# GAIR-Lab/IISAN

Measured on AMD Instinct MI355X. Metric: items/s (fwd+bwd) ViT-B+BERT-B IISAN uncached, Scientific, bs=128, higher is better.
Workload: dtype fp16; 1 GPU; Code_Uncached IISAN ViT-base+BERT-base, Amazon-Scientific-shaped synthetic batch, bs=128/GPU (1408 item slots, all encoded), 1xMI355X per rank; global_batch=128, parallelism=dp1, encoder_blocks=all tokens in every block

## Files before the change

### iisan_amd/csrc/attn16.hip

```cpp
#include "common.h"
#ifndef ATTN_KBATCH
#define ATTN_KBATCH 4
#endif

#ifdef ATTN_DEBUG_BITS
static int g_attn_dbg = 0;
IISAN_DEV_KNOB(attn_debug, g_attn_dbg);
#else
static constexpr int g_attn_dbg = 0;
#endif

namespace {

constexpr float MASK_RAW = -0x1p126f;

template <typename T> struct Mfma16k16;
template <> struct Mfma16k16<F16> {
    static __device__ __forceinline__ f4 run(h4 a, h4 b, f4 c) { return __builtin_amdgcn_mfma_f32_16x16x16f16(a, b, c, 0, 0, 0); }
};
template <> struct Mfma16k16<BF16> {
    typedef short s4 __attribute__((ext_vector_type(4)));
    static __device__ __forceinline__ f4 run(b4 a, b4 b, f4 c) {
        return __builtin_amdgcn_mfma_f32_16x16x16bf16_1k(__builtin_bit_cast(s4, a), __builtin_bit_cast(s4, b), c, 0, 0, 0);
    }
};

template <typename T, int NT16, bool PF, bool MASKALL>
__global__ __launch_bounds__(256, PF ? 2 : 3) void attention16_kernel(const typename T::elem* __restrict__ qkv,
                                                             const float* __restrict__ key_bias,
                                                             typename T::elem* __restrict__ ctx, int S, int heads, int hpw,
                                                             int dbg_arg) {
    typedef typename T::elem E;
    typedef typename T::v8 V8;
    typedef typename T::v4 V4;
#ifndef ATTN_DEBUG_BITS
    (void)dbg_arg;
    constexpr int dbg = 0;
#else
    const int dbg = dbg_arg;
#endif
    constexpr int SP = NT16 * 16;
    constexpr int VT_LD = 32 * ((NT16 + 1) / 2) + 16;
    constexpr int MAXQB = (NT16 + 3) / 4;
    constexpr int KP = (SP + 31) / 32;
    constexpr int VP = (SP / 4 + 31) / 32;
    __shared__ __attribute__((aligned(16))) char smem[SP * 128 + 64 * VT_LD * 2 + SP * 4];
    char* sK = smem;
    E* sVt = (E*)(smem + SP * 128);
    float* sKB = (float*)(smem + SP * 128 + 64 * VT_LD * 2);

    const int tid = threadIdx.x, lane = tid & 63, wave = tid >> 6;
    const int groups = heads / hpw;
    const int item = blockIdx.x / groups, h0 = (blockIdx.x - item * groups) * hpw;
    const int D = heads * 64;
    const int j = lane & 15, g = lane >> 4;
    const int nqb = (S + 15) >> 4;
    const int c = tid & 7, r0 = tid >> 3;

    V8 kreg[KP], vreg[VP][4], qnext[MAXQB][2];
    auto load_head = [&](int h) {
        if (dbg & 32) return;
        const E* qb_ = qkv + ((int64_t)item * heads + h) * 3 * S * 64;
        const E* kb_ = qb_ + (int64_t)S * 64;
        const E* vb_ = kb_ + (int64_t)S * 64;
        int t2 = tid;
        asm volatile("" : "+v"(t2));
        const int wave = t2 >> 6, j = t2 & 15, g = (t2 >> 4) & 3, c = t2 & 7, r0 = t2 >> 3;
#pragma unroll
        for (int i = 0; i < MAXQB; ++i) {
            int sq = (wave + 4 * i) * 16 + j;
            sq = sq < S ? sq : S - 1;
#pragma unroll
            for (int kk = 0; kk < 2; ++kk) qnext[i][kk] = *(const V8*)(qb_ + (unsigned)(sq * 64 + kk * 32 + g * 8));
        }
#pragma unroll
        for (int p = 0; p < KP; ++p) {
            const int r = r0 + 32 * p;
            kreg[p] = __builtin_nontemporal_load((const V8*)(kb_ + (unsigned)((r < S ? r : S - 1) * 64 + c * 8)));
        }
#pragma unroll
        for (int p = 0; p < VP; ++p)
#pragma unroll
            for (int r = 0; r < 4; ++r) {
                const int key = (r0 + 32 * p) * 4 + r;
                if (SP > 64 || r0 + 32 * p < SP / 4) vreg[p][r] = __builtin_nontemporal_load((const V8*)(vb_ + (unsigned)((key < S ? key : S - 1) * 64 + c * 8)));
            }
    };

    if (PF) load_head(h0);
    for (int r = tid; r < SP; r += 256)
        sKB[r] = r >= S ? -INFINITY : ((key_bias && key_bias[(int64_t)item * S + r] < 0.f) ? MASK_RAW : INFINITY);

    const float c2 = 0.18033688011112042f;
#pragma unroll 1
    for (int hi = 0; hi < hpw; ++hi) {
        const int h = h0 + hi;
        if (!PF) load_head(h);
        if (hi > 0) __syncthreads();
#pragma unroll
        for (int p = 0; p < KP; ++p) {
            const int r = r0 + 32 * p;
            if ((SP % 32 == 0 || r < SP) && !(dbg & 16)) *(V8*)(sK + r * 128 + ((c ^ (r & 7)) << 4)) = kreg[p];
        }
#pragma unroll
        for (int p = 0; p < VP; ++p) {
            const int kg = r0 + 32 * p;
            if (kg < SP / 4) {
#pragma unroll
                for (int e = 0; e < 8; ++e) {
                    V4 t;
#pragma unroll
                    for (int r = 0; r < 4; ++r) t[r] = vreg[p][r][e];
                    if (!(dbg & 1)) *(V4*)(sVt + (c * 8 + e) * VT_LD + 32 * (kg >> 3) + 8 * (kg & 3) + 4 * ((kg >> 2) & 1)) = t;
                }
            }
        }
        V8 qf[MAXQB][2];
#pragma unroll
        for (int i = 0; i < MAXQB; ++i)
#pragma unroll
            for (int kk = 0; kk < 2; ++kk) qf[i][kk] = qnext[i][kk];
        __syncthreads();
        if (PF && hi + 1 < hpw) load_head(h + 1);

#pragma unroll
        for (int i = 0; i < MAXQB; ++i) {
            const int qb = wave + 4 * i;
            if (qb >= nqb || (dbg & 64)) break;
            const int sq = qb * 16 + j;

            f4 sc[NT16];
            {
                constexpr int KBATCH = NT16 >= 13 ? ATTN_KBATCH : (NT16 % 4 == 0 ? 4 : NT16);
#pragma unroll
                for (int t0 = 0; t0 < NT16; t0 += KBATCH) {
                    V8 kf[KBATCH][2];
#pragma unroll
                    for (int u = 0; u < KBATCH; ++u)
#pragma unroll
                        for (int kk = 0; kk < 2; ++kk)
                            if (t0 + u < NT16) kf[u][kk] = *(const V8*)(sK + ((t0 + u) * 16 + j) * 128 + (((kk * 4 + g) ^ (j & 7)) << 4));
                    __builtin_amdgcn_sched_barrier(0);
#pragma unroll
                    for (int u = 0; u < KBATCH; ++u) {
                        if (t0 + u >= NT16) continue;
                        f4 acc = {0.f, 0.f, 0.f, 0.f};
                        acc = T::mfma(kf[u][0], qf[i][0], acc);
                        acc = T::mfma(kf[u][1], qf[i][1], acc);
                        sc[t0 + u] = acc;
                    }
                }
            }
#pragma unroll
            for (int t = 0; t < NT16; ++t) {
                if (MASKALL || t == NT16 - 1) {
                    const f4 kb = *(const f4*)(sKB + t * 16 + g * 4);
#pragma unroll
                    for (int r = 0; r < 4; ++r) sc[t][r] = __builtin_amdgcn_fmed3f(sc[t][r], kb[r], -INFINITY);
                }
            }
            float mx0 = -INFINITY, mx1 = -INFINITY;
#pragma unroll
            for (int t = 0; t < NT16; ++t) {
                if (t & 1) mx1 = fmaxf(fmaxf(mx1, sc[t][0]), fmaxf(sc[t][1], fmaxf(sc[t][2], sc[t][3])));
                else mx0 = fmaxf(fmaxf(mx0, sc[t][0]), fmaxf(sc[t][1], fmaxf(sc[t][2], sc[t][3])));
            }
            float mx = fmaxf(mx0, mx1);
            mx = fmaxf(mx, __shfl_xor(mx, 16, 64));
            mx = fmaxf(mx, __shfl_xor(mx, 32, 64));
            f4 sum4 = {0.f, 0.f, 0.f, 0.f};
            const float mxs = -(mx * c2);
#pragma unroll
            for (int t = 0; t < NT16; ++t)
#pragma unroll
                for (int r = 0; r < 4; ++r) {
                    const float a = fmaf(sc[t][r], c2, mxs);
                    const float p = __builtin_amdgcn_exp2f(a);
                    sc[t][r] = p;
                    sum4[r] += p;
                }
            float sum = (sum4[0] + sum4[1]) + (sum4[2] + sum4[3]);
            sum += __shfl_xor(sum, 16, 64);
            sum += __shfl_xor(sum, 32, 64);
            const float inv = 1.0f / sum;

            f4 o[4];
#pragma unroll
            for (int dt = 0; dt < 4; ++dt) o[dt] = (f4){0.f, 0.f, 0.f, 0.f};
            {
                auto vload = [&](int kb, V8 (&vf)[4]) {
#pragma unroll
                    for (int dt = 0; dt < 4; ++dt) vf[dt] = *(const V8*)(sVt + (dt * 16 + j) * VT_LD + kb * 32 + g * 8);
                };
                V8 vc[4];
                vload(0, vc);
                constexpr int NPV = NT16 / 2;
#pragma unroll
                for (int kb = 0; kb < NPV; ++kb) {
                    V8 vn[4];
                    if (kb + 1 < NPV) vload(kb + 1, vn);
                    V8 pf;
#pragma unroll
                    for (int e = 0; e < 4; ++e) {
                        pf[e] = T::from_f32(sc[2 * kb][e]);
                        pf[4 + e] = T::from_f32(sc[2 * kb + 1][e]);
                    }
#pragma unroll
                    for (int dt = 0; dt < 4; ++dt) o[dt] = T::mfma(vc[dt], pf, o[dt]);
                    if (kb + 1 < NPV) {
#pragma unroll
                        for (int dt = 0; dt < 4; ++dt) vc[dt] = vn[dt];
                    }
                }
                if constexpr (NT16 % 2 == 1) {
                    V4 pt;
#pragma unroll
                    for (int e = 0; e < 4; ++e) pt[e] = T::from_f32(sc[NT16 - 1][e]);
#pragma unroll
                    for (int dt = 0; dt < 4; ++dt)
                        o[dt] = Mfma16k16<T>::run(*(const V4*)(sVt + (dt * 16 + j) * VT_LD + (NT16 / 2) * 32 + g * 8), pt, o[dt]);
                }
            }
            typedef unsigned u2 __attribute__((ext_vector_type(2)));
            u2 pk[4];
#pragma unroll
            for (int dt = 0; dt < 4; ++dt) {
                V4 ov;
#pragma unroll
                for (int r = 0; r < 4; ++r) ov[r] = T::from_f32(o[dt][r] * inv);
                pk[dt] = __builtin_bit_cast(u2, ov);
            }
#pragma unroll
            for (int q2 = 0; q2 < 2; ++q2)
#pragma unroll
                for (int w = 0; w < 2; ++w) {
                    const auto sw = __builtin_amdgcn_permlane16_swap(pk[2 * q2][w], pk[2 * q2 + 1][w], false, false);
                    pk[2 * q2][w] = sw[0];
                    pk[2 * q2 + 1][w] = sw[1];
                }
            if (sq < S && !(dbg & 8)) {
                int g2 = g;
                asm volatile("" : "+v"(g2));
                E* op = ctx + (size_t)item * S * D + (unsigned)(sq * D + h * 64 + g2 * 4 + ((g2 & 1) ? 12 : 0));
                typedef unsigned u4 __attribute__((ext_vector_type(4)));
#pragma unroll
                for (int q2 = 0; q2 < 2; ++q2)
                    *(u4*)(op + q2 * 32) = (u4){pk[2 * q2][0], pk[2 * q2][1], pk[2 * q2 + 1][0], pk[2 * q2 + 1][1]};
            }
        }
    }
}

template <typename T>
__global__ __launch_bounds__(256) void attention_cls_kernel(const typename T::elem* __restrict__ qkv,
                                                            const float* __restrict__ key_bias,
                                                            typename T::elem* __restrict__ ctx, int64_t pairs, int S, int heads,
                                                            const typename T::elem* __restrict__ q_cls) {
    typedef typename T::elem E;
    typedef typename T::v8 V8;
    typedef typename T::v4 V4;
    __shared__ float sP[4][256];
    const int lane = threadIdx.x & 63, wave = threadIdx.x >> 6;
    const int64_t pair = (int64_t)blockIdx.x * 4 + wave;
    if (pair >= pairs) return;
    const int64_t item = pair / heads;
    const int h = (int)(pair - item * heads);
    const E* qb_ = qkv + pair * 3 * S * 64;
    const E* kb_ = qb_ + (int64_t)S * 64;
    const E* vb_ = kb_ + (int64_t)S * 64;
    const int kc = lane & 7, kr = lane >> 3;
    float q[8];
    {
        const V8 t = q_cls ? *(const V8*)(q_cls + (item * heads + h) * 64 + kc * 8) : *(const V8*)(qb_ + kc * 8);
#pragma unroll
        for (int e = 0; e < 8; ++e) q[e] = T::to_f32(t[e]);
    }
    float mx = -INFINITY;
    constexpr int KB = 5;
    for (int k0 = 0; k0 < S; k0 += 8 * KB) {
        V8 t[KB];
        float kbv[KB];
#pragma unroll
        for (int u = 0; u < KB; ++u) {
            const int key = k0 + 8 * u + kr;
            const int kcl = key < S ? key : S - 1;
            t[u] = *(const V8*)(kb_ + (int64_t)kcl * 64 + kc * 8);
            kbv[u] = key_bias ? key_bias[item * S + kcl] : 0.f;
        }
#pragma unroll
        for (int u = 0; u < KB; ++u) {
            const int key = k0 + 8 * u + kr;
            float a = 0.f;
#pragma unroll
            for (int e = 0; e < 8; ++e) a = fmaf(q[e], T::to_f32(t[u][e]), a);
            a += __shfl_xor(a, 1, 64);
            a += __shfl_xor(a, 2, 64);
            a += __shfl_xor(a, 4, 64);
            if (key >= S) a = -INFINITY;
            else if (kbv[u] < 0.f) a = MASK_RAW;
            if (kc == 0 && key < 256) sP[wave][key] = a;
            mx = fmaxf(mx, a);
        }
    }
#pragma unroll
    for (int o = 8; o < 64; o <<= 1) mx = fmaxf(mx, __shfl_xor(mx, o, 64));
    __builtin_amdgcn_s_waitcnt(0xc07f);
    const float c2 = 0.18033688011112042f;
    float sum = 0.f;
#pragma unroll
    for (int i = 0; i < 4; ++i) {
        const int key = lane + 64 * i;
        const float a = key < S ? sP[wave][key] : -INFINITY;
        const float p = __builtin_amdgcn_exp2f((a - mx) * c2);
        sum += p;
        sP[wave][key] = T::to_f32(T::from_f32(p));
    }
#pragma unroll
    for (int o = 1; o < 64; o <<= 1) sum += __shfl_xor(sum, o, 64);
    const float inv = 1.0f / sum;
    __builtin_amdgcn_s_waitcnt(0xc07f);
    const int kg = lane >> 4, dq = lane & 15;
    float acc[4] = {0.f, 0.f, 0.f, 0.f};
    constexpr int VB = 8;
    for (int k0 = kg; k0 < S; k0 += 4 * VB) {
        V4 v[VB];
        float pr[VB];
#pragma unroll
        for (int u = 0; u < VB; ++u) {
            const int key = k0 + 4 * u;
            const int kcl = key < S ? key : S - 1;
            v[u] = *(const V4*)(vb_ + (int64_t)kcl * 64 + dq * 4);
            pr[u] = key < S ? sP[wave][kcl] : 0.f;
        }
#pragma unroll
        for (int u = 0; u < VB; ++u)
#pragma unroll
            for (int e = 0; e < 4; ++e) acc[e] = fmaf(pr[u], T::to_f32(v[u][e]), acc[e]);
    }
#pragma unroll
    for (int e = 0; e < 4; ++e) {
        acc[e] += __shfl_xor(acc[e], 16, 64);
        acc[e] += __shfl_xor(acc[e], 32, 64);
    }
    if (kg == 0) {
        V4 o;
#pragma unroll
        for (int e = 0; e < 4; ++e) o[e] = T::from_f32(acc[e] * inv);
        *(V4*)(ctx + item * (int64_t)heads * 64 + h * 64 + dq * 4) = o;
    }
}

template <typename T>
int launch_t(const void* qkv, const float* key_bias, void* ctx, int64_t items, int S, int heads, hipStream_t s) {
    typedef typename T::elem E;
    int hpw = heads % 2 == 0 ? 2 : 1;
#ifdef ATTN_DEBUG_BITS
    {
        const int want = (g_attn_dbg >> 8) & 15;
        if (want > 0 && heads % want == 0) hpw = want;
    }
#endif
    dim3 grid((unsigned)(items * (heads / hpw))), block(256);
#define IISAN_ATTN_CASE(NT)                                                                                                       \
    if (key_bias == nullptr && S > 16 * (NT - 1))                                                                                 \
        hipLaunchKernelGGL((attention16_kernel<T, NT, true, false>), grid, block, 0, s, (const E*)qkv, key_bias, (E*)ctx, S, heads, hpw, g_attn_dbg & 127); \
    else                                                                                                                          \
        hipLaunchKernelGGL((attention16_kernel<T, NT, true, true>), grid, block, 0, s, (const E*)qkv, key_bias, (E*)ctx, S, heads, hpw, g_attn_dbg & 127)
    if (S <= 32) { IISAN_ATTN_CASE(2); }
    else if (S <= 64) { IISAN_ATTN_CASE(4); }
    else if (S <= 128) { IISAN_ATTN_CASE(8); }
    else if (S <= 208) { IISAN_ATTN_CASE(13); }
    else if (S <= 224) { IISAN_ATTN_CASE(14); }
    else {
        iisan_set_error("attention16: sequence length %d > 224 not supported", S);
        return IISAN_EBADSHAPE;
    }
#undef IISAN_ATTN_CASE
    IISAN_LAUNCH_OK();
    return IISAN_OK;
}

}

int launch_attention16(int dtype16, const void* qkv, const float* key_bias, void* ctx, int64_t items, int S, int heads,
                       hipStream_t s) {
    IISAN_CHECK_SHAPE(items > 0 && S > 0 && heads > 0, "attention16: empty problem");
    IISAN_CHECK_SHAPE(items * heads < (1ll << 31), "attention16: grid too large");
    IISAN_CHECK_SHAPE((int64_t)S * heads * 64 < (1ll << 31), "attention16: item of %d x %d elements too large", S, heads * 64);
    return dtype16 == IISAN_BF16 ? launch_t<BF16>(qkv, key_bias, ctx, items, S, heads, s)
                                 : launch_t<F16>(qkv, key_bias, ctx, items, S, heads, s);
}

int launch_attention_cls16(int dtype16, const void* qkv, const float* key_bias, void* ctx_cls, int64_t items, int S, int heads,
                           hipStream_t s, const void* q_cls) {
    IISAN_CHECK_SHAPE(items > 0 && S > 0 && S <= 256 && heads > 0, "attention_cls16: unsupported problem (S=%d)", S);
    const int64_t pairs = items * heads;
    dim3 grid((unsigned)ceil_div(pairs, 4)), block(256);
    if (dtype16 == IISAN_BF16)
        hipLaunchKernelGGL(attention_cls_kernel<BF16>, grid, block, 0, s, (const __bf16*)qkv, key_bias, (__bf16*)ctx_cls, pairs, S, heads, (const __bf16*)q_cls);
    else
        hipLaunchKernelGGL(attention_cls_kernel<F16>, grid, block, 0, s, (const _Float16*)qkv, key_bias, (_Float16*)ctx_cls, pairs, S, heads, (const _Float16*)q_cls);
    IISAN_LAUNCH_OK();
    return IISAN_OK;
}

extern "C" int iisan_attention16(int32_t dtype16, const void* qkv, const float* key_bias, void* ctx, int64_t items,
                                 int32_t S, int32_t heads, void* stream) {
    return launch_attention16(dtype16, qkv, key_bias, ctx, items, S, heads, (hipStream_t)stream);
}

extern "C" int iisan_attention_cls16(int32_t dtype16, const void* qkv, const float* key_bias, void* ctx_cls, int64_t items,
                                     int32_t S, int32_t heads, void* stream) {
    return launch_attention_cls16(dtype16, qkv, key_bias, ctx_cls, items, S, heads, (hipStream_t)stream, nullptr);
}
```

### iisan_amd/csrc/common.h

```cpp
#pragma once

#include <hip/hip_runtime.h>
#include <stdint.h>
#include <stdio.h>
#include <string.h>

#include "../../include/iisan_hip.h"

typedef _Float16 h8 __attribute__((ext_vector_type(8)));
typedef _Float16 h4 __attribute__((ext_vector_type(4)));
typedef __bf16 b8 __attribute__((ext_vector_type(8)));
typedef __bf16 b4 __attribute__((ext_vector_type(4)));
typedef float f4 __attribute__((ext_vector_type(4)));
typedef unsigned int u4 __attribute__((ext_vector_type(4)));
typedef unsigned int u2 __attribute__((ext_vector_type(2)));

#define WAVE 64

void iisan_set_error(const char* fmt, ...);

#define IISAN_CHECK_SHAPE(cond, ...)                                                                             \
    do {                                                                                                         \
        if (!(cond)) {                                                                                           \
            iisan_set_error(__VA_ARGS__);                                                                        \
            return IISAN_EBADSHAPE;                                                                              \
        }                                                                                                        \
    } while (0)

#define IISAN_HIP_OK(expr)                                                                                       \
    do {                                                                                                         \
        hipError_t _e = (expr);                                                                                  \
        if (_e != hipSuccess) {                                                                                  \
            iisan_set_error("%s failed at %s:%d: %s", #expr, __FILE__, __LINE__, hipGetErrorString(_e));         \
            return IISAN_EHIP;                                                                                   \
        }                                                                                                        \
    } while (0)

#define IISAN_LAUNCH_OK() IISAN_HIP_OK(hipGetLastError())

struct IisanDevKnob {
    const char* name;
    int64_t def;
    int64_t (*get)();
    void (*set)(int64_t);
};
int iisan_dev_register(const IisanDevKnob& k);
#define IISAN_DEV_KNOB(NAME, VAR)                                                                                \
    static const int iisan_dev_reg_##NAME = iisan_dev_register(IisanDevKnob{                                     \
        #NAME, (int64_t)(VAR), [] { return (int64_t)(VAR); }, [](int64_t v) { VAR = (decltype(VAR))v; }})
#define IISAN_DEV_COUNTER(NAME, VAR)                                                                             \
    static const int iisan_dev_cnt_##NAME = iisan_dev_register(IisanDevKnob{                                     \
        "count:" #NAME, INT64_MIN, [] { return (int64_t)(VAR); }, [](int64_t v) { VAR = (decltype(VAR))v; }})
#define IISAN_DEV_KNOB_FN(NAME, VAR, SET)                                                                        \
    static const int iisan_dev_reg_##NAME = iisan_dev_register(IisanDevKnob{                                     \
        #NAME, (int64_t)(VAR), [] { return (int64_t)(VAR); }, [](int64_t v) { SET; }})

#define IISAN_TRY(expr)                                                                                          \
    do {                                                                                                         \
        int _r = (expr);                                                                                         \
        if (_r != IISAN_OK) return _r;                                                                           \
    } while (0)

constexpr int IISAN_MAX_DEVICES = 64;
int iisan_cu_count();
struct OncePerDevice {
    bool done[IISAN_MAX_DEVICES] = {};
    bool first() {
        int dev = 0;
        if (hipGetDevice(&dev) != hipSuccess || dev < 0 || dev >= IISAN_MAX_DEVICES) return true;
        if (done[dev]) return false;
        done[dev] = true;
        return true;
    }
};

static inline size_t align_up(size_t x, size_t a) { return (x + a - 1) / a * a; }
static inline int64_t ceil_div(int64_t a, int64_t b) { return (a + b - 1) / b; }

struct WsCarver {
    char* base;
    size_t cap, off;
    bool overflow;
    WsCarver(void* p, size_t n) : base((char*)p), cap(n), off(0), overflow(false) {}
    template <typename T>
    T* take(size_t count) {
        size_t bytes = align_up(count * sizeof(T), 256);
        if (base && off + bytes > cap) overflow = true;
        T* r = base ? (T*)(base + off) : nullptr;
        off += bytes;
        return r;
    }
};

struct F16 {
    typedef _Float16 elem;
    typedef h8 v8;
    typedef h4 v4;
    static __device__ __forceinline__ f4 mfma(v8 a, v8 b, f4 c) {
        return __builtin_amdgcn_mfma_f32_16x16x32_f16(a, b, c, 0, 0, 0);
    }
    static __device__ __forceinline__ elem from_f32(float x) { return (_Float16)x; }
    static __device__ __forceinline__ float to_f32(elem x) { return (float)x; }
};
struct BF16 {
    typedef __bf16 elem;
    typedef b8 v8;
    typedef b4 v4;
    static __device__ __forceinline__ f4 mfma(v8 a, v8 b, f4 c) {
        return __builtin_amdgcn_mfma_f32_16x16x32_bf16(a, b, c, 0, 0, 0);
    }
    static __device__ __forceinline__ elem from_f32(float x) { return (__bf16)x; }
    static __device__ __forceinline__ float to_f32(elem x) { return (float)x; }
};

__device__ __forceinline__ float wave_sum(float v) {
#pragma unroll
    for (int o = 32; o > 0; o >>= 1) v += __shfl_xor(v, o, 64);
    return v;
}
__device__ __forceinline__ float wave_max(float v) {
#pragma unroll
    for (int o = 32; o > 0; o >>= 1) v = fmaxf(v, __shfl_xor(v, o, 64));
    return v;
}
__device__ __forceinline__ float gelu_erf(float x) { return 0.5f * x * (1.0f + erff(x * 0.70710678118654752440f)); }
constexpr float GELU_X0 = 5.5f;
__device__ __forceinline__ float gelu_absmin(float x) {
    float r;
    asm("v_min_f32 %0, |%1|, %2" : "=v"(r) : "v"(x), "v"(GELU_X0));
    return r;
}
__device__ __forceinline__ float gelu_relu(float x) {
    float r;
    asm("v_max_f32 %0, 0, %1" : "=v"(r) : "v"(x));
    return r;
}
constexpr float GELU_C0 = 9.170038104e-01f, GELU_C1 = -9.149338305e-02f, GELU_C2 = -3.171720356e-02f, GELU_C3 = -1.111552469e-03f,
                GELU_C4 = 1.940784161e-03f, GELU_C5 = -1.910830324e-04f;
__device__ __forceinline__ float gelu_erf_fast(float x) {
    const float a = gelu_absmin(x);
    float p = fmaf(a, GELU_C5, GELU_C4);
    p = fmaf(p, a, GELU_C3);
    p = fmaf(p, a, GELU_C2);
    p = fmaf(p, a, GELU_C1);
    p = fmaf(p, a, GELU_C0);
    p = p * p; p = p * p; p = p * p;
    return fmaf(-a, p, gelu_relu(x));
}
typedef float f2 __attribute__((ext_vector_type(2)));
template <int NP>
__device__ __forceinline__ void gelu_erf_fast2xN(f2* x) {
    f2 a[NP], p[NP];
#pragma unroll
    for (int k = 0; k < NP; ++k) { a[k][0] = gelu_absmin(x[k][0]); a[k][1] = gelu_absmin(x[k][1]); }
#pragma unroll
    for (int k = 0; k < NP; ++k) p[k] = __builtin_elementwise_fma(a[k], (f2)GELU_C5, (f2)GELU_C4);
#pragma unroll
    for (int k = 0; k < NP; ++k) p[k] = __builtin_elementwise_fma(p[k], a[k], (f2)GELU_C3);
#pragma unroll
    for (int k = 0; k < NP; ++k) p[k] = __builtin_elementwise_fma(p[k], a[k], (f2)GELU_C2);
#pragma unroll
    for (int k = 0; k < NP; ++k) p[k] = __builtin_elementwise_fma(p[k], a[k], (f2)GELU_C1);
#pragma unroll
    for (int k = 0; k < NP; ++k) p[k] = __builtin_elementwise_fma(p[k], a[k], (f2)GELU_C0);
#pragma unroll
    for (int sq = 0; sq < 3; ++sq)
#pragma unroll
        for (int k = 0; k < NP; ++k) p[k] = p[k] * p[k];
#pragma unroll
    for (int k = 0; k < NP; ++k) {
        f2 mx;
        mx[0] = gelu_relu(x[k][0]); mx[1] = gelu_relu(x[k][1]);
        x[k] = __builtin_elementwise_fma(-a[k], p[k], mx);
    }
}
__device__ __forceinline__ void gelu_erf_fast2x8(f2 (&x)[8]) { gelu_erf_fast2xN<8>(x); }
__device__ __forceinline__ float gelu_erf_grad(float x) {
    const float cdf = 0.5f * (1.0f + erff(x * 0.70710678118654752440f));
    const float pdf = 0.39894228040143267794f * __expf(-0.5f * x * x);
    return cdf + x * pdf;
}

__device__ __forceinline__ float drop_scale(uint64_t seed, uint32_t site, uint64_t idx, uint32_t thr24, float inv_keep) {
    uint64_t x = seed + (uint64_t)site * 0x9E3779B97F4A7C15ull + idx * 0xD1B54A32D192ED03ull;
    x ^= x >> 32; x *= 0xD6E8FEB86659FD93ull;
    x ^= x >> 32; x *= 0xD6E8FEB86659FD93ull;
    x ^= x >> 32;
    return ((uint32_t)(x >> 8) & 0xFFFFFFu) >= thr24 ? inv_keep : 0.f;
}
struct DropCfg {
    uint64_t seed;
    uint32_t site, thr24;
    float inv_keep;
};
static inline DropCfg make_drop(uint64_t seed, uint32_t site, float p) {
    DropCfg d;
    d.seed = seed; d.site = site;
    d.thr24 = p > 0.f ? (uint32_t)(p * 16777216.0f) : 0u;
    d.inv_keep = p > 0.f ? 1.0f / (1.0f - p) : 1.0f;
    return d;
}

__device__ __forceinline__ void glds16(const void* gsrc, void* lds_wave_base) {
    __builtin_amdgcn_global_load_lds((const __attribute__((address_space(1))) void*)gsrc,
                                     (__attribute__((address_space(3))) void*)lds_wave_base, 16, 0, 0);
}

__device__ __forceinline__ int xcd_remap(int bid, int nwg) {
    const int q = nwg >> 3, r = nwg & 7;
    const int xcd = bid & 7, idx = bid >> 3;
    return (xcd < r ? xcd * (q + 1) : r * (q + 1) + (xcd - r) * q) + idx;
}

bool iisan_timing_on(hipStream_t s);
int iisan_timing_class();
void iisan_timing_pre(hipStream_t s, double flops, double bytes);
void iisan_timing_post(hipStream_t s);
inline thread_local int iisan_timing_depth = 0;
struct TimedLaunch {
    hipStream_t s; int cls; bool on;
    TimedLaunch(int cls_, hipStream_t s_, double flops, double bytes)
        : s(s_), cls(cls_), on(cls_ == 1 ? iisan_timing_on(s_) : iisan_timing_class() == 2 && iisan_timing_depth == 0) {
        if (cls == 2) ++iisan_timing_depth;
        if (on) iisan_timing_pre(s, flops, bytes);
    }
    ~TimedLaunch() {
        if (cls == 2) --iisan_timing_depth;
        if (on) iisan_timing_post(s);
    }
};

struct Gemm16Args {
    const void* A;
    const void* W;
    const float* bias;
    void* out;
    const float* resid;
    const float* pos;
    int64_t M;
    int32_t N, K;
    int32_t lda, ldw, ldo;
    int32_t patch_P;
    int32_t qkv_S, qkv_heads;
    int32_t qkv_which0;
    int32_t debug;
    int32_t walk_c, walk_h;
    const float* rowstat;
    float* rowpart;
    const float* inv_a; const float* inv_b;
    int32_t atomic;
    int64_t split_stride;
    const int32_t* skip_last_third;
};
enum { EPI_OUT16 = 0, EPI_GELU16 = 1, EPI_RESID32 = 2, EPI_PATCH32 = 3, EPI_QKVH16 = 4, EPI_F32 = 5, EPI_PATCH16 = 6, EPI_STREAM16 = 7 };
int launch_gemm16(int dtype16, int mode, const Gemm16Args& a, hipStream_t s);
enum { G16_REJECTED = -1, G16_V1 = 0, G16_S256 = 1, G16_H256 = 2 };
int gemm16_route(int dtype16, int mode, const Gemm16Args& a);
bool gemm16_s256_applicable(int mode, const Gemm16Args& a);
int launch_gemm16_s256(int dtype16, int mode, const Gemm16Args& a, hipStream_t s);
bool gemm16_h256_applicable(int mode, const Gemm16Args& a);
int launch_gemm16_h256(int dtype16, int mode, const Gemm16Args& a, hipStream_t s);
int launch_gemm16_f32(const Gemm16Args& a, int ksplit, hipStream_t s);
int launch_layernorm768(int dtype16, const float* x, const float* g, const float* b, float eps, void* out16,
                        float* out32, int64_t rows, hipStream_t s);
int launch_add_layernorm768(int dtype16, const float* x, const void* delta16, const float* g, const float* b, float eps,
                            float* sum32, void* out16, float* out32, int64_t rows, hipStream_t s);
int launch_add2_layernorm768(int dtype16, const float* x, const void* delta16, const void* delta16b, const float* g,
                             const float* b, float eps, float* sum32, void* out16, float* out32, int64_t rows, hipStream_t s);
enum { MX_D1 = 1, MX_D2 = 2, MX_LN = 4, MX_RESV = 8, MX_RESY = 16, MX_SRC32 = 32, MX_CLSONLY = 64, MX_POSROW = 128, MX_STAT = 256, MX_ALIAS = 512 };
int launch_layernorm768_mixed(int dtype16, int V, const float* x32, void* x16, float* xc, const void* delta16, const void* delta16b,
                              const float* g, const float* b, float eps, void* out16, int64_t items, int Ttok, hipStream_t s,
                              float* stat = nullptr);
struct LnFoldJob { const void* W; const float* bias; const float* g; const float* b; void* Wf; float* bf; int32_t N;
                   int32_t w32;
};
int launch_fold_ln_weights(const LnFoldJob* jobs, int n, hipStream_t s);
int launch_stream_stats_finalize(const float* rowpart, int nslots, int64_t Mpad, void* x16, float* xc, float* rstat, float eps,
                                 int64_t items, int Ttok, hipStream_t s);
int launch_attention16(int dtype16, const void* qkv, const float* key_bias, void* ctx, int64_t items, int S,
                       int heads, hipStream_t s);
int launch_attention_cls16(int dtype16, const void* qkv, const float* key_bias, void* ctx_cls, int64_t items, int S,
                           int heads, hipStream_t s, const void* q_cls = nullptr);
int launch_vit_im2col(int dtype16, const void* img, int img_u8, void* out, int64_t M, int C, int R, int p, hipStream_t s);
int launch_vit_im2col_indexed(int dtype16, const uint8_t* catalogue, int64_t rows, const int64_t* index, void* out, int64_t M, int C,
                              int R, int p, hipStream_t s);
int launch_vit_cls_rows(float* X, const float* cls, const float* pos, int64_t M, int T, int D, hipStream_t s);
int launch_bert_embed_ln(int dtype16, const int64_t* text, const float* word, const float* pos, const float* type0,
                         const float* g, const float* b, float eps, float* X, void* H, float* key_bias, int64_t M,
                         int W, int vocab, hipStream_t s, void* X16 = nullptr, float* Xc = nullptr);
int launch_bert_embed_ln_indexed(int dtype16, const int64_t* table, int64_t rows, const int64_t* index, const float* word, const float* pos,
                                 const float* type0, const float* g, const float* b, float eps, float* X, void* H, float* key_bias,
                                 int64_t M, int W, int vocab, hipStream_t s, void* X16 = nullptr, float* Xc = nullptr);
int launch_gather_cls(const float* X, float* taps, int64_t M, int T, int D, int n_taps, int k, hipStream_t s);
int launch_gather_rows16(const void* H, void* out, int64_t M, int T, int D, hipStream_t s);

struct Gemm32Prob;
size_t gemm_x3_ws_bytes(int64_t M, int64_t N, int64_t K);
bool gemm_x3_applicable(const Gemm32Prob& p, int flags);
int launch_gemm_x3(const Gemm32Prob& p, int flags, void* ws, size_t ws_bytes, hipStream_t s);
size_t gemm_x3_group_ws_bytes(const int64_t* M, const int64_t* N, const int64_t* K, int n);
int launch_gemm_x3_group(const Gemm32Prob* probs, int n, int flags, void* ws, size_t ws_bytes, hipStream_t s);
int gemm_x3_group_max();
double gemm_x3_get_min_flops();
void gemm_x3_set_min_flops(double f);

struct X3pArgs {
    const _Float16* A2; const _Float16* B2;
    int64_t M; int32_t N, kp;
    const float* bias; const float* resid; float* out; int32_t ldo;
    const float* inv_a; const float* inv_b;
    const int32_t* lo_a; const int32_t* lo_b;
    int64_t split_stride;
};
int launch_gemm16_x3p(const X3pArgs& a, int ksplit, hipStream_t s);
int x3p_tile_n(int64_t M, int64_t N);

struct AmaxBatch { const float* x[16]; int64_t rows[16], cols[16], ld[16]; uint32_t* out[16]; };
int launch_amax_batch(const AmaxBatch& b, int n, hipStream_t s);

struct FuseOperands {
    const float* a; const float* b; const float* prev;
    int64_t lda, ldb, ldp;
    const float* gate;
    int32_t D, type;
};
struct Gemm32Prob {
    const float* A; const float* B; const float* bias; const float* resid; const float* act_src; float* C;
    int64_t M; int32_t N; int64_t K;
    int32_t lda, ldb, ldc, ldr;
    DropCfg drop;
    int64_t ksplit_stride;
    uint32_t* amax_a; uint32_t* amax_b;
    int32_t amax_a_ready, amax_b_ready;
    int32_t exact16_a, exact16_b;
    uint32_t* x3_zeroed;
    float* colsum_a;
};
struct N64FDesc {
    FuseOperands f;
    float* F;
    const float* W; int32_t ldw;
    const float* bias;
    float* U; float* A;
    int64_t M; int32_t K;
};
bool gemm32_n64f_ok(const N64FDesc* d, int n);
int launch_gemm32_n64f(const N64FDesc* d, int n, int gelu, hipStream_t s);
struct K64Gate { const float* gate; const float* ga; const float* go; int64_t ldga, ldgo; float* dgate; int32_t scale_prev, store; float* d2; int64_t ldd2; int32_t d2_is_b; };
bool gemm32_k64_gate_ok(const Gemm32Prob* probs, const K64Gate* gates, int nprob);
int launch_gemm32_k64_gate(const Gemm32Prob* probs, const K64Gate* gates, int nprob, hipStream_t s);
void gemm32_set_scratch(float* ws, size_t floats);
enum {
    G32_TA = 1,
    G32_TB = 2,
    G32_RELU = 4,
    G32_GELU = 8,
    G32_ACCUM = 16,
    G32_MUL_RELU_MASK = 32,
    G32_MUL_GELU_GRAD = 64,
    G32_PREACT = 128,
    G32_HINT_B_EXACT16 = 1024,
    G32_DROPOUT = 256,
};
int launch_gemm32(const Gemm32Prob* probs, int nprob, int flags, hipStream_t s);
int launch_colsum(const float* const* X, float* const* out, const int64_t* M, const int32_t* N, const int32_t* ld,
                  int nprob, hipStream_t s);

struct SanbTowerDesc {
    FuseOperands f;
    const float* Wd; const float* bd; const float* Wu; const float* bu;
    float* F; float* U; float* A; float* O;
    const float* dO; const float* Upre; float* dU; float* dprev; float* da; float* db; float* dgate; float* dbu; float* dbd;
};
bool sanb_fused_ok(int D, int down);
int launch_sanb_fwd(const SanbTowerDesc* towers, int n, int64_t M, int gelu, hipStream_t s);
int launch_sanb_bwd(const SanbTowerDesc* towers, int n, int64_t M, int gelu, hipStream_t s);
int launch_sanb_transpose(const float* const* in, float* const* out, const int32_t* rows, const int32_t* cols, int n, hipStream_t s);

struct SasFusedPtrs {
    float* Z0; float* X0;
    float* Q[8]; float* K[8]; float* V[8]; float* P[8]; float* C[8]; float* Zattn[8]; float* X1[8]; float* Hf[8]; float* Zffn[8]; float* X2[8];
};
bool sasrec_fused_ok(const iisan_sasrec_cfg* cfg);
bool sasrec_fused_shape_ok(const iisan_sasrec_cfg* cfg);
int launch_sasrec_fused_fwd(const iisan_sasrec_cfg* cfg, const float* x, const float* log_mask, int64_t B, const void* const* params,
                            float* y, const SasFusedPtrs& w, hipStream_t s);
int64_t sasrec_fused_slab_floats(const iisan_sasrec_cfg* cfg, int64_t B);
int launch_sasrec_fused_bwd(const iisan_sasrec_cfg* cfg, const float* log_mask, int64_t B, const void* const* params, const float* dy,
                            float* dx, void* const* grads, const SasFusedPtrs& w, float* slab, hipStream_t s);
```

Baseline: 22860 items/s.

## Add dedicated ViT attention kernel with LDS-staged K/V and cross-head prefetch

Adds a specialised attention kernel for ViT sequence lengths (193..224, no key mask). It stages K and V tiles into LDS through direct global-to-LDS loads with swizzled layouts, and reads V with transposing LDS loads. It double-buffers K across heads so the next head's K and Q loads overlap the current head's softmax and PV MFMAs. The existing attention launcher routes to it by default, at the cost of extra hand-scheduled code using inline asm, waitcnt and permlane swaps.

```diff
diff --git a/iisan_amd/csrc/attn16.hip b/iisan_amd/csrc/attn16.hip
--- a/iisan_amd/csrc/attn16.hip
+++ b/iisan_amd/csrc/attn16.hip
@@ -353,6 +353,8 @@
 template <typename T>
 int launch_t(const void* qkv, const float* key_bias, void* ctx, int64_t items, int S, int heads, hipStream_t s) {
     typedef typename T::elem E;
+    if (key_bias == nullptr && S > 192 && S <= 224 && attention_vit_enabled())
+        return launch_attention_vit(__is_same(T, BF16) ? IISAN_BF16 : IISAN_F16, qkv, ctx, items, S, heads, s);
     int hpw = heads % 2 == 0 ? 2 : 1;
 #ifdef ATTN_DEBUG_BITS
     {
diff --git a/iisan_amd/csrc/attn16_vit.hip b/iisan_amd/csrc/attn16_vit.hip
--- /dev/null
+++ b/iisan_amd/csrc/attn16_vit.hip
@@ -0,0 +1,328 @@
+#include "common.h"
+#include <type_traits>
+
+static int g_attn_vit = 1;
+IISAN_DEV_KNOB(attn_vit, g_attn_vit);
+
+namespace {
+
+#define AV_FENCE() __builtin_amdgcn_sched_barrier(0)
+#define AV_BARRIER()                                 \
+    do {                                             \
+        AV_FENCE();                                  \
+        asm volatile("s_barrier" ::: "memory");      \
+        AV_FENCE();                                  \
+    } while (0)
+#define AV_VMCNT(n)                                                                                \
+    do {                                                                                           \
+        AV_FENCE();                                                                                \
+        __builtin_amdgcn_s_waitcnt(((n) & 15) | (7 << 4) | (15 << 8) | ((((n) >> 4) & 3) << 14));  \
+        AV_FENCE();                                                                                \
+    } while (0)
+
+typedef __fp16 hf4 __attribute__((ext_vector_type(4)));
+#define AV_LDS __attribute__((address_space(3)))
+
+template <typename T> struct MfmaK16;
+template <> struct MfmaK16<F16> {
+    static __device__ __forceinline__ f4 run(h4 a, h4 b, f4 c) { return __builtin_amdgcn_mfma_f32_16x16x16f16(a, b, c, 0, 0, 0); }
+};
+template <> struct MfmaK16<BF16> {
+    typedef short s4 __attribute__((ext_vector_type(4)));
+    static __device__ __forceinline__ f4 run(b4 a, b4 b, f4 c) {
+        return __builtin_amdgcn_mfma_f32_16x16x16bf16_1k(__builtin_bit_cast(s4, a), __builtin_bit_cast(s4, b), c, 0, 0, 0);
+    }
+};
+
+__device__ __forceinline__ void swap16(float& a, float& b) {
+    asm volatile("s_nop 1\n\tv_permlane16_swap_b32 %0, %1\n\ts_nop 1" : "+v"(a), "+v"(b));
+}
+__device__ __forceinline__ void swap32(float& a, float& b) {
+    asm volatile("s_nop 1\n\tv_permlane32_swap_b32 %0, %1\n\ts_nop 1" : "+v"(a), "+v"(b));
+}
+__device__ __forceinline__ float quad_max(float x) {
+    float a = x, b = x;
+    swap16(a, b);
+    a = fmaxf(a, b);
+    b = a;
+    swap32(a, b);
+    return fmaxf(a, b);
+}
+__device__ __forceinline__ float quad_sum(float x) {
+    float a = x, b = x;
+    swap16(a, b);
+    a = a + b;
+    b = a;
+    swap32(a, b);
+    return a + b;
+}
+
+template <typename T, int NT16>
+__global__ __launch_bounds__(256, 2) void attention_vit_kernel(const typename T::elem* __restrict__ qkv, typename T::elem* __restrict__ ctx,
+                                                              int S, int heads, int hpw) {
+    typedef typename T::elem E;
+    typedef typename T::v8 V8;
+    typedef typename T::v4 V4;
+    constexpr int SP = NT16 * 16;
+    constexpr int TILE = SP * 128;
+    constexpr int NG = SP / 8;
+    constexpr int AV_NDMA = (NG + 3) / 4;
+    extern __shared__ __attribute__((aligned(16))) char smem[];
+
+    const int tid = threadIdx.x, lane = tid & 63;
+    const int wave = __builtin_amdgcn_readfirstlane(tid >> 6);
+    const int groups = heads / hpw;
+    const int item = blockIdx.x / groups, h0 = (blockIdx.x - item * groups) * hpw;
+    const int D = heads * 64;
+    const int j = lane & 15, g = lane >> 4;
+
+    auto dma = [&](const E* src, bool v_image, int lds_off) {
+        int l2 = lane;
+        asm volatile("" : "+v"(l2));
+        const int drow = l2 >> 3;
+        const int col = v_image ? (((((l2 & 7) >> 1) ^ ((l2 >> 4) & 3)) << 1) | (l2 & 1)) * 8 : ((l2 & 7) ^ drow) * 8;
+#pragma unroll
+        for (int i = 0; i < AV_NDMA; ++i) {
+            int grp = wave + 4 * i;
+            if (4 * i + 3 >= NG) grp = grp < NG ? grp : NG - 1;
+            int r = grp * 8 + drow;
+            r = r < S ? r : S - 1;
+            glds16(src + (unsigned)(r * 64 + col), smem + lds_off + grp * 1024);
+        }
+    };
+    auto head_ptr = [&](int h) { return qkv + ((int64_t)item * heads + h) * 3 * S * 64; };
+    auto load_q = [&](const E* qb_, int pair, V8 (&q)[2][2]) {
+        int l2 = lane;
+        asm volatile("" : "+v"(l2));
+        const int j = l2 & 15, g = l2 >> 4;
+#pragma unroll
+        for (int b = 0; b < 2; ++b) {
+            int sq = (2 * pair + b) * 16 + j;
+            sq = sq < S ? sq : S - 1;
+#pragma unroll
+            for (int kk = 0; kk < 2; ++kk) q[b][kk] = *(const V8*)(qb_ + (unsigned)(sq * 64 + kk * 32 + g * 8));
+        }
+    };
+
+    const int koff = j * 128 + ((g ^ (j & 7)) << 4);
+    int voff[4];
+    {
+        const int row = 4 * g + (j >> 2), sw = (row >> 1) & 3;
+#pragma unroll
+        for (int dt = 0; dt < 4; ++dt) voff[dt] = 2 * TILE + row * 128 + ((dt ^ sw) << 5) + 8 * (j & 3);
+    }
+    auto vtr = [&](int dt, int byte_off) {
+        return __builtin_bit_cast(V4, __builtin_amdgcn_ds_read_tr16_b64_v4f16((AV_LDS hf4*)(smem + voff[dt] + byte_off)));
+    };
+
+    const float c2 = 0.18033688011112042f;
+
+    V8 q0[2][2], q1[2][2];
+    auto run_pair = [&](auto nbc, auto midc, const V8 (&q)[2][2], int pair, int h, bool next, bool last, const char* sK) {
+        constexpr int NB = decltype(nbc)::value;
+        constexpr bool MID = decltype(midc)::value;
+        f4 sc[NB][NT16];
+        {
+            constexpr int KBT = 2;
+            V8 kc[KBT][2], kn[KBT][2];
+            auto kload = [&](int t0, V8 (&kf)[KBT][2]) {
+#pragma unroll
+                for (int u = 0; u < KBT; ++u)
+#pragma unroll
+                    for (int kk = 0; kk < 2; ++kk)
+                        if (t0 + u < NT16) kf[u][kk] = *(const V8*)(sK + (t0 + u) * 2048 + (koff ^ (kk << 6)));
+            };
+            kload(0, kc);
+#pragma unroll
+            for (int t0 = 0; t0 < NT16; t0 += KBT) {
+                if (t0 + KBT < NT16) kload(t0 + KBT, kn);
+                AV_FENCE();
+#pragma unroll
+                for (int u = 0; u < KBT; ++u) {
+                    if (t0 + u >= NT16) continue;
+#pragma unroll
+                    for (int b = 0; b < NB; ++b) {
+                        f4 acc = {0.f, 0.f, 0.f, 0.f};
+                        acc = T::mfma(kc[u][0], q[b][0], acc);
+                        acc = T::mfma(kc[u][1], q[b][1], acc);
+                        sc[b][t0 + u] = acc;
+                    }
+                }
+                if (t0 + KBT < NT16) {
+#pragma unroll
+                    for (int u = 0; u < KBT; ++u)
+#pragma unroll
+                        for (int kk = 0; kk < 2; ++kk) kc[u][kk] = kn[u][kk];
+                }
+            }
+        }
+        float inv[NB];
+#pragma unroll
+        for (int b = 0; b < NB; ++b) {
+#pragma unroll
+            for (int r = 0; r < 4; ++r) sc[b][NT16 - 1][r] = (NT16 - 1) * 16 + 4 * g + r < S ? sc[b][NT16 - 1][r] : -INFINITY;
+            float mx0 = -INFINITY, mx1 = -INFINITY;
+#pragma unroll
+            for (int t = 0; t < NT16; ++t) {
+                if (t & 1) mx1 = fmaxf(fmaxf(mx1, sc[b][t][0]), fmaxf(sc[b][t][1], fmaxf(sc[b][t][2], sc[b][t][3])));
+                else mx0 = fmaxf(fmaxf(mx0, sc[b][t][0]), fmaxf(sc[b][t][1], fmaxf(sc[b][t][2], sc[b][t][3])));
+            }
+            const float mx = quad_max(fmaxf(mx0, mx1));
+            const float mxs = -(mx * c2);
+            float s0 = 0.f, s1 = 0.f;
+#pragma unroll
+            for (int t = 0; t < NT16; ++t)
+#pragma unroll
+                for (int r = 0; r < 4; ++r) {
+                    const float p = __builtin_amdgcn_exp2f(fmaf(sc[b][t][r], c2, mxs));
+                    sc[b][t][r] = p;
+                    if (t & 1) s1 += p;
+                    else s0 += p;
+                }
+            inv[b] = 1.0f / quad_sum(s0 + s1);
+        }
+        if constexpr (MID) {
+            if (next) {
+                AV_FENCE();
+                load_q(head_ptr(h + 1), wave, q0);
+                AV_VMCNT(AV_NDMA + 4);
+            } else
+                AV_VMCNT(0);
+            AV_BARRIER();
+        }
+
+        f4 o[NB][4];
+#pragma unroll
+        for (int b = 0; b < NB; ++b)
+#pragma unroll
+            for (int dt = 0; dt < 4; ++dt) o[b][dt] = (f4){0.f, 0.f, 0.f, 0.f};
+        {
+            constexpr int NPV = NT16 / 2;
+            auto vload = [&](int kb, V8 (&vf)[4]) {
+#pragma unroll
+                for (int dt = 0; dt < 4; ++dt)
+                    vf[dt] = __builtin_shufflevector(vtr(dt, kb * 4096), vtr(dt, kb * 4096 + 2048), 0, 1, 2, 3, 4, 5, 6, 7);
+            };
+            V8 vc[4], vn[4];
+            V4 vt[4];
+            vload(0, vc);
+#pragma unroll
+            for (int kb = 0; kb < NPV; ++kb) {
+                if (kb + 1 < NPV) vload(kb + 1, vn);
+                else if constexpr (NT16 % 2 == 1) {
+#pragma unroll
+                    for (int dt = 0; dt < 4; ++dt) vt[dt] = vtr(dt, NPV * 4096);
+                }
+                AV_FENCE();
+#pragma unroll
+                for (int b = 0; b < NB; ++b) {
+                    V8 pf;
+#pragma unroll
+                    for (int e = 0; e < 4; ++e) {
+                        pf[e] = T::from_f32(sc[b][2 * kb][e]);
+                        pf[4 + e] = T::from_f32(sc[b][2 * kb + 1][e]);
+                    }
+#pragma unroll
+                    for (int dt = 0; dt < 4; ++dt) o[b][dt] = T::mfma(vc[dt], pf, o[b][dt]);
+                }
+                if (kb + 1 < NPV) {
+#pragma unroll
+                    for (int dt = 0; dt < 4; ++dt) vc[dt] = vn[dt];
+                }
+            }
+            if constexpr (NT16 % 2 == 1) {
+#pragma unroll
+                for (int b = 0; b < NB; ++b) {
+                    V4 pt;
+#pragma unroll
+                    for (int e = 0; e < 4; ++e) pt[e] = T::from_f32(sc[b][NT16 - 1][e]);
+#pragma unroll
+                    for (int dt = 0; dt < 4; ++dt) o[b][dt] = MfmaK16<T>::run(vt[dt], pt, o[b][dt]);
+                }
+            }
+        }
+        if (last && next) AV_VMCNT(0);
+#pragma unroll
+        for (int b = 0; b < NB; ++b) {
+            u2 pk[4];
+#pragma unroll
+            for (int dt = 0; dt < 4; ++dt) {
+                V4 ov;
+#pragma unroll
+                for (int r = 0; r < 4; ++r) ov[r] = T::from_f32(o[b][dt][r] * inv[b]);
+                pk[dt] = __builtin_bit_cast(u2, ov);
+            }
+#pragma unroll
+            for (int q2 = 0; q2 < 2; ++q2)
+#pragma unroll
+                for (int w = 0; w < 2; ++w) {
+                    const auto sw = __builtin_amdgcn_permlane16_swap(pk[2 * q2][w], pk[2 * q2 + 1][w], false, false);
+                    pk[2 * q2][w] = sw[0];
+                    pk[2 * q2 + 1][w] = sw[1];
+                }
+            const int sq = (2 * pair + b) * 16 + j;
+            if (sq < S) {
+                int g2 = g;
+                asm volatile("" : "+v"(g2));
+                E* op = ctx + (size_t)item * S * D + (unsigned)(sq * D + h * 64 + g2 * 4 + ((g2 & 1) ? 12 : 0));
+#pragma unroll
+                for (int q2 = 0; q2 < 2; ++q2) *(u4*)(op + q2 * 32) = (u4){pk[2 * q2][0], pk[2 * q2][1], pk[2 * q2 + 1][0], pk[2 * q2 + 1][1]};
+            }
+        }
+    };
+
+    const bool has_p1 = wave < 3;
+    {
+        const E* hp = head_ptr(h0);
+        load_q(hp, wave, q0);
+        AV_FENCE();
+        dma(hp + (int64_t)S * 64, false, 0);
+        dma(hp + (int64_t)2 * S * 64, true, 2 * TILE);
+        AV_VMCNT(AV_NDMA);
+        AV_BARRIER();
+    }
+#pragma unroll 1
+    for (int hi = 0; hi < hpw; ++hi) {
+        const int h = h0 + hi;
+        const bool next = hi + 1 < hpw;
+        const char* sK = smem + (hi & 1) * TILE;
+        if (has_p1) load_q(head_ptr(h), wave + 4, q1);
+        AV_FENCE();
+        if (next) dma(head_ptr(h + 1) + (int64_t)S * 64, false, ((hi + 1) & 1) * TILE);
+        AV_FENCE();
+        run_pair(std::integral_constant<int, 2>{}, std::true_type{}, q0, wave, h, next, !has_p1, sK);
+        if (has_p1) {
+            if (NT16 % 2 == 1 && wave == 2) run_pair(std::integral_constant<int, 1>{}, std::false_type{}, q1, wave + 4, h, next, true, sK);
+            else run_pair(std::integral_constant<int, 2>{}, std::false_type{}, q1, wave + 4, h, next, true, sK);
+        }
+        if (next) {
+            AV_BARRIER();
+            dma(head_ptr(h + 1) + (int64_t)2 * S * 64, true, 2 * TILE);
+        }
+    }
+}
+
+template <typename T, int NT16>
+int launch_nt(const void* qkv, void* ctx, int64_t items, int S, int heads, int hpw, hipStream_t s) {
+    typedef typename T::elem E;
+    static OncePerDevice attr;
+    auto kern = attention_vit_kernel<T, NT16>;
+    constexpr int LDS = 3 * NT16 * 16 * 128;
+    if (attr.first()) IISAN_HIP_OK(hipFuncSetAttribute((const void*)kern, hipFuncAttributeMaxDynamicSharedMemorySize, LDS));
+    hipLaunchKernelGGL(kern, dim3((unsigned)(items * (heads / hpw))), dim3(256), LDS, s, (const E*)qkv, (E*)ctx, S, heads, hpw);
+    IISAN_LAUNCH_OK();
+    return IISAN_OK;
+}
+
+}
+
+bool attention_vit_enabled() { return g_attn_vit != 0; }
+
+int launch_attention_vit(int dtype16, const void* qkv, void* ctx, int64_t items, int S, int heads, hipStream_t s) {
+    IISAN_CHECK_SHAPE(S > 192 && S <= 224, "attention_vit: sequence length %d outside 193..224", S);
+    int hpw = heads % 2 == 0 ? 2 : 1;
+    if (g_attn_vit >= 2 && heads % g_attn_vit == 0) hpw = g_attn_vit;
+    if (dtype16 == IISAN_BF16)
+        return S <= 208 ? launch_nt<BF16, 13>(qkv, ctx, items, S, heads, hpw, s) : launch_nt<BF16, 14>(qkv, ctx, items, S, heads, hpw, s);
+    return S <= 208 ? launch_nt<F16, 13>(qkv, ctx, items, S, heads, hpw, s) : launch_nt<F16, 14>(qkv, ctx, items, S, heads, hpw, s);
+}
diff --git a/iisan_amd/csrc/common.h b/iisan_amd/csrc/common.h
--- a/iisan_amd/csrc/common.h
+++ b/iisan_amd/csrc/common.h
@@ -279,6 +279,8 @@
                                  int64_t items, int Ttok, hipStream_t s);
 int launch_attention16(int dtype16, const void* qkv, const float* key_bias, void* ctx, int64_t items, int S,
                        int heads, hipStream_t s);
+bool attention_vit_enabled();
+int launch_attention_vit(int dtype16, const void* qkv, void* ctx, int64_t items, int S, int heads, hipStream_t s);
 int launch_attention_cls16(int dtype16, const void* qkv, const float* key_bias, void* ctx_cls, int64_t items, int S,
                            int heads, hipStream_t s, const void* q_cls = nullptr);
 int launch_vit_im2col(int dtype16, const void* img, int img_u8, void* out, int64_t M, int C, int R, int p, hipStream_t s);
```

After: 23060 items/s, median of 6. No clear change (+0.9%).
